# Wionerlol/MultimodalEmotionRecognition

Measured on AMD Instinct MI355X. Metric: 3s-clip train steps/sec (B=32, xattn fusion) at 1/2/4/8 MI355X, higher is better.
Workload: dtype bf16; 1 GPU; ResNet18 + WavLM-base (frozen) + xattn fusion train step (fwd+bwd+Adam); per_gpu_batch=32, global_batch=32, frames=8, image=112, audio_samples=48000, parallelism=dp1

## Files before the change

### include/mer.h

```cpp
#ifndef MER_H_
#define MER_H_

#define MER_BN_STAT_PARTS 64
#define MER_BN_STAT_ROWS(M) (((M) + 63) / 64 + 64)
#define MER_BN_RED_ROWS(M) (((M) + 63) / 64 + 4 + 64)
#define MER_BN_RED_WS_ROWS 576

#ifdef __cplusplus
extern "C" {
#endif


int mer_gemm_f32(int M, int N, int K, const void* A, int a_dtype, long sam, long sak, long bsa, const void* B,
                 int b_dtype, long sbk, long sbn, long bsb, float* C, long ldc, long bsc, const float* bias, int beta,
                 int act, int splitk, int batch, float* workspace, void* stream);

#define MER_COLSUM_WS_FLOATS(M, N) ((long)(((M) + 15) / 16) * (N))
int mer_colsum_f32(int M, int N, const float* X, long ldx, float* out, float* workspace, void* stream);

int mer_mha_fwd(int B, int H, int Lq, int Lk, int dh, const float* Q, long ldq, const float* K, long ldk,
                const float* V, long ldv, const float* bias, float* O, long ldo, float* P, float scale, float drop_p,
                const unsigned long long* seed, unsigned long long site, void* stream);

int mer_mha_bwd(int B, int H, int Lq, int Lk, int dh, const float* Q, long ldq, const float* K, long ldk,
// ... 162 lines not shown


int mer_conv_fwd(int N, int H, int W, int C, int K, int R, int S, int stride, int pad, const void* x,
                 const void* w_packed, void* y, float* stats, void* stream);

int mer_conv_fwd_ex(int N, int H, int W, int C, int K, int R, int S, int stride, int pad, const void* x,
                    const void* w_packed, void* y, float* stats, int variant, void* stream);

int mer_conv_dgrad(int N, int H, int W, int C, int K, int R, int S, int stride, int pad, const void* dy,
                   const void* wt_packed, void* dx, const void* residual, const void* residual_mask, void* stream);
int mer_conv_dgrad_ex(int N, int H, int W, int C, int K, int R, int S, int stride, int pad, const void* dy,
                      const void* wt_packed, void* dx, const void* residual, const void* residual_mask, int variant,
                      void* stream);

int mer_conv_dgrad_bnr(int N, int H, int W, int C, int K, int R, int S, int stride, int pad, const void* dy,
                       const void* wt_packed, void* dx, const void* residual, const void* residual_mask,
                       const void* bn_mask, const void* bn_x, const float* bn_ms, float* bn_red, const void* bn_x2,
                       const float* bn_ms2, float* bn_red2, int variant, void* stream);
int mer_conv_dgrad_ds(int N, int H, int W, int C, int K, int R, int S, int stride, int pad, const void* dy,
                      const void* wt_packed, void* dx, const void* residual, const void* residual_mask,
                      const void* bn_mask, const void* bn_x, const float* bn_ms, float* bn_red, const void* bn_x2,
                      const float* bn_ms2, float* bn_red2, const void* ds_dy, const void* ds_wt_packed, int ds_K,
                      int variant, void* stream);

int mer_conv_fwd_rows(int N, int H, int W, int C, int K, int R, int S, int stride, int pad, const void* x,
                      const void* w_packed, int variant);
int mer_conv_dgrad_rows(int N, int H, int W, int C, int K, int R, int S, int stride, int pad, const void* dy,
                        const void* wt_packed, const void* ds_dy, int variant);

int mer_partials_sum(int C, int parts, float* in, float* out, void* stream);
int mer_partials_sum2(int C, int parts, float* in, float* out, float* in2, float* out2, void* stream);

int mer_conv_wgrad(int N, int H, int W, int C, int Creal, int K, int R, int S, int stride, int pad, const void* x,
                   const void* dy, float* dw, int splits, float* workspace, void* stream);
int mer_conv_wgrad_ex(int N, int H, int W, int C, int Creal, int K, int R, int S, int stride, int pad, const void* x,
                      const void* dy, float* dw, int splits, float* workspace, int variant, void* stream);
int mer_conv_wgrad_partials(int N, int H, int W, int C, int K, int R, int S, int stride, int pad, const void* x,
                            const void* dy, int splits, float* workspace, int variant, void* stream);
int mer_wgrad_fold_batch(int n, const long long* rows, void* stream);

int mer_pack_input_nhwc(int N, int C, int H, int W, int Cp, const float* x, void* y, void* stream);
int mer_pack_input_s2d(int N, int C, int H, int W, const float* x, void* y, void* stream);

int mer_pack_conv_weight(int K, int C, int R, int S, int Cp, int transpose, const float* w, void* out, void* stream);

int mer_pack_conv_weights(int n, const long long* desc, long total, void* stream);
// ... 139 lines not shown
```

### multimodalemotionrecognition_amd/csrc/bn_pool.hip

```cpp
#include "common.h"
#include "mer.h"

typedef __attribute__((ext_vector_type(4))) uint32_t u32x4;

__global__ __launch_bounds__(256) void bn_stat_rows_fold_kernel(int C2, int rows, int per, const float* __restrict__ in,
                                                                float* __restrict__ out) {
  __shared__ float part[4][64];
  const int el = threadIdx.x & 63, pg = threadIdx.x >> 6;
  const int e = blockIdx.x * 64 + el, grp = blockIdx.y;
  const int r0 = grp * per, r1 = min(rows, r0 + per);
  const int ec = e < C2 ? e : C2 - 1;
  const int n = r1 - (r0 + pg) > 0 ? (r1 - (r0 + pg) + 3) / 4 : 0;
  float a0 = 0.f, a1 = 0.f;
  for (int i0 = 0; i0 < n; i0 += 16) {
    float x[16];
#pragma unroll
    for (int i = 0; i < 16; ++i) {
      const int r = r0 + pg + 4 * (i0 + i);
      x[i] = in[(long)(r < r1 ? r : r1 - 1) * C2 + ec];
    }
#pragma unroll
    for (int i = 0; i < 16; i += 2) {
      if (i0 + i < n) a0 += x[i];
      if (i0 + i + 1 < n) a1 += x[i + 1];
// ... 565 lines not shown
        float* db = h ? dbeta2 : dbeta;
        if (dg) dg[c] += rd[2 * c + 1];
        if (db) db[c] += rd[2 * c];
      }
      const float mu = m[2 * c], rs = m[2 * c + 1], gr = (h ? gamma2 : gamma)[c] * rs;
      const float a = batch_stats ? rd[2 * c] * invM : 0.f;
      const float b = batch_stats ? rd[2 * c + 1] * invM : 0.f;
      const float t = gr * b * rs;
      coef[3 * h + 0][c] = gr;
      coef[3 * h + 1][c] = -t;
      coef[3 * h + 2][c] = fmaf(-gr, a, t * mu);
    }
  }
  __syncthreads();
  const long nvec = M * C / 8;
  const long stride = (long)gridDim.x * blockDim.x;
  const long tid0 = blockIdx.x * (long)blockDim.x + threadIdx.x;
  const int c0 = (int)(tid0 % (C / 8)) * 8;
  float k[6][8];
#pragma unroll
  for (int j = 0; j < 6; ++j)
#pragma unroll
    for (int i = 0; i < 8; ++i) k[j][i] = coef[j][c0 + i];
  for (long e = tid0; e < nvec; e += stride) {
    const u32x4 gv = *reinterpret_cast<const u32x4*>(dy + e * 8);
    const u32x4 mv = *reinterpret_cast<const u32x4*>(mask + e * 8);
    const u32x4 xv = *reinterpret_cast<const u32x4*>(x + e * 8);
    const u32x4 x2v = *reinterpret_cast<const u32x4*>(x2 + e * 8);
    const bf16_t* gh = reinterpret_cast<const bf16_t*>(&gv);
    const bf16_t* mh = reinterpret_cast<const bf16_t*>(&mv);
    const bf16_t* xh = reinterpret_cast<const bf16_t*>(&xv);
    const bf16_t* x2h = reinterpret_cast<const bf16_t*>(&x2v);
    u32x4 ov, o2v;
    bf16_t* oh = reinterpret_cast<bf16_t*>(&ov);
    bf16_t* o2h = reinterpret_cast<bf16_t*>(&o2v);
#pragma unroll
    for (int i = 0; i < 8; ++i) {
      const float g = bf2f(mh[i]) > 0.f ? bf2f(gh[i]) : 0.f;
      oh[i] = f2bf(fmaf(k[0][i], g, fmaf(k[1][i], bf2f(xh[i]), k[2][i])));
      o2h[i] = f2bf(fmaf(k[3][i], g, fmaf(k[4][i], bf2f(x2h[i]), k[5][i])));
    }
    *reinterpret_cast<u32x4*>(dx + e * 8) = ov;
    *reinterpret_cast<u32x4*>(dx2 + e * 8) = o2v;
  }
}
MER_API int mer_bn_bwd_apply2(long M, int C, const void* dy, const void* mask, const void* x, const float* ms,
                              const float* gamma, const float* red, const void* x2, const float* ms2,
                              const float* gamma2, const float* red2, int batch_stats, void* dx, void* dx2,
                              float* dgamma, float* dbeta, float* dgamma2, float* dbeta2, void* stream) {
  if (C % 8 || C > 512 || 256 % (C / 8) || !mask || !x2 || !dx2 || dx == dy || dx2 == dy)
    return (int)hipErrorInvalidValue;
  const long nvec = M * C / 8;
  const int grid = bn_stream_grid(nvec);
  hipLaunchKernelGGL(bn_bwd_apply2_kernel, dim3(grid), dim3(256), 0, (hipStream_t)stream, M, C, (const bf16_t*)dy,
                     (const bf16_t*)mask, (const bf16_t*)x, ms, gamma, red, (const bf16_t*)x2, ms2, gamma2, red2,
                     batch_stats, (bf16_t*)dx, (bf16_t*)dx2, dgamma, dbeta, dgamma2, dbeta2);
  MER_LAUNCH_CHECK();
}

__global__ void maxpool_fwd_kernel(int N, int H, int W, int C, int Ho, int Wo, const bf16_t* __restrict__ x,
                                   bf16_t* __restrict__ y, uint8_t* __restrict__ arg) {
  const int cpr = C / 8;
  const int total = N * Ho * Wo * cpr;
  const float inv_cpr = 1.f / cpr, inv_Wo = 1.f / Wo, inv_Ho = 1.f / Ho;
  for (int e = blockIdx.x * blockDim.x + threadIdx.x; e < total; e += gridDim.x * blockDim.x) {
    const int q = fdiv(e, inv_cpr);
    const int c0 = (e - q * cpr) * 8;
    const int q2 = fdiv(q, inv_Wo);
    const int ow = q - q2 * Wo;
    const int n = fdiv(q2, inv_Ho);
    const int oh = q2 - n * Ho;
    float best[8];
    int bi[8];
// ... 10 lines not shown
          const float f = bf2f(vh[i]);
          if (f > best[i]) { best[i] = f; bi[i] = r * 3 + s; }
        }
      }
    u32x4 o;
    bf16_t* oh8 = reinterpret_cast<bf16_t*>(&o);
    uint2 a;
    uint8_t* a8 = reinterpret_cast<uint8_t*>(&a);
#pragma unroll
    for (int i = 0; i < 8; ++i) { oh8[i] = f2bf(best[i]); a8[i] = (uint8_t)bi[i]; }
    *reinterpret_cast<u32x4*>(y + (long)q * C + c0) = o;
    *reinterpret_cast<uint2*>(arg + (long)q * C + c0) = a;
  }
}
MER_API int mer_maxpool_fwd(int N, int H, int W, int C, const void* x, void* y, void* argmax, void* stream) {
  const int Ho = (H + 2 - 3) / 2 + 1, Wo = (W + 2 - 3) / 2 + 1;
  if (C % 8 || (long)N * H * W >= (1L << 22)) return (int)hipErrorInvalidValue;
  const long total = (long)N * Ho * Wo * C / 8;
  const int grid = (int)((total + 255) / 256 < 8192 ? (total + 255) / 256 : 8192);
  hipLaunchKernelGGL(maxpool_fwd_kernel, dim3(grid), dim3(256), 0, (hipStream_t)stream, N, H, W, C, Ho, Wo,
                     (const bf16_t*)x, (bf16_t*)y, (uint8_t*)argmax);
  MER_LAUNCH_CHECK();
}
__global__ void maxpool_bwd_kernel(int N, int H, int W, int C, int Ho, int Wo, const bf16_t* __restrict__ dy,
                                   const uint8_t* __restrict__ arg, bf16_t* __restrict__ dx) {
  const int cpr = C / 8;
  const int total = N * H * W * cpr;
  const float inv_cpr = 1.f / cpr, inv_W = 1.f / W, inv_H = 1.f / H;
  for (int e = blockIdx.x * blockDim.x + threadIdx.x; e < total; e += gridDim.x * blockDim.x) {
    const int q = fdiv(e, inv_cpr);
    const int c0 = (e - q * cpr) * 8;
    const int q2 = fdiv(q, inv_W);
    const int w = q - q2 * W;
    const int n = fdiv(q2, inv_H);
    const int h = q2 - n * H;
    float acc[8] = {0.f, 0.f, 0.f, 0.f, 0.f, 0.f, 0.f, 0.f};
    u32x4 gq[2][2];
    uint2 aq[2][2];
    int tap[2][2];
#pragma unroll
    for (int a = 0; a < 2; ++a)
#pragma unroll
      for (int b = 0; b < 2; ++b) {
        const int oh = (h + 1) / 2 - 1 + a, ow = (w + 1) / 2 - 1 + b;
        const int r = h - (oh * 2 - 1), s = w - (ow * 2 - 1);
        const bool ok = oh >= 0 && oh < Ho && ow >= 0 && ow < Wo && r >= 0 && r <= 2 && s >= 0 && s <= 2;
        const int ohc = oh < 0 ? 0 : (oh >= Ho ? Ho - 1 : oh), owc = ow < 0 ? 0 : (ow >= Wo ? Wo - 1 : ow);
        const long oi = (((long)n * Ho + ohc) * Wo + owc) * C + c0;
        gq[a][b] = *reinterpret_cast<const u32x4*>(dy + oi);
        aq[a][b] = *reinterpret_cast<const uint2*>(arg + oi);
        tap[a][b] = ok ? r * 3 + s : -1;
      }
#pragma unroll
    for (int a = 0; a < 2; ++a)
#pragma unroll
      for (int b = 0; b < 2; ++b) {
        const bf16_t* gh = reinterpret_cast<const bf16_t*>(&gq[a][b]);
        const uint8_t* a8 = reinterpret_cast<const uint8_t*>(&aq[a][b]);
#pragma unroll
        for (int i = 0; i < 8; ++i)
          if ((int)a8[i] == tap[a][b]) acc[i] += bf2f(gh[i]);
      }
    u32x4 o;
    bf16_t* oh8 = reinterpret_cast<bf16_t*>(&o);
#pragma unroll
    for (int i = 0; i < 8; ++i) oh8[i] = f2bf(acc[i]);
    *reinterpret_cast<u32x4*>(dx + (long)q * C + c0) = o;
  }
}
MER_API int mer_maxpool_bwd(int N, int H, int W, int C, const void* dy, const void* argmax, void* dx, void* stream) {
  const int Ho = (H + 2 - 3) / 2 + 1, Wo = (W + 2 - 3) / 2 + 1;
  if (C % 8 || (long)N * H * W >= (1L << 22)) return (int)hipErrorInvalidValue;
  const long total = (long)N * H * W * C / 8;
  const int grid = (int)((total + 255) / 256 < 8192 ? (total + 255) / 256 : 8192);
  hipLaunchKernelGGL(maxpool_bwd_kernel, dim3(grid), dim3(256), 0, (hipStream_t)stream, N, H, W, C, Ho, Wo,
                     (const bf16_t*)dy, (const uint8_t*)argmax, (bf16_t*)dx);
  MER_LAUNCH_CHECK();
}


__global__ void stem_bnrelu_maxpool_kernel(int N, int H, int W, int C, int Ho, int Wo, const bf16_t* __restrict__ x,
                                           const float* __restrict__ ms, const float* __restrict__ gamma,
                                           const float* __restrict__ beta, bf16_t* __restrict__ y,
                                           uint8_t* __restrict__ arg) {
  const int cpr = C / 8;
  const int total = N * Ho * Wo * cpr;
  const float inv_cpr = 1.f / cpr, inv_Wo = 1.f / Wo, inv_Ho = 1.f / Ho;
  for (int e = blockIdx.x * blockDim.x + threadIdx.x; e < total; e += gridDim.x * blockDim.x) {
    const int q = fdiv(e, inv_cpr);
// ... 30 lines not shown
    }
    u32x4 o;
    bf16_t* oh8 = reinterpret_cast<bf16_t*>(&o);
    uint2 a;
    uint8_t* a8 = reinterpret_cast<uint8_t*>(&a);
#pragma unroll
    for (int i = 0; i < 8; ++i) { oh8[i] = f2bf(best[i]); a8[i] = (uint8_t)bi[i]; }
    *reinterpret_cast<u32x4*>(y + (long)q * C + c0) = o;
    *reinterpret_cast<uint2*>(arg + (long)q * C + c0) = a;
  }
}

MER_API int mer_stem_bnrelu_maxpool_fwd(int N, int H, int W, int C, const void* x, const float* ms, const float* gamma,
                                        const float* beta, void* y, void* argmax, void* stream) {
  const int Ho = (H + 2 - 3) / 2 + 1, Wo = (W + 2 - 3) / 2 + 1;
  if (C % 8 || C > 512 || (long)N * H * W >= (1L << 22)) return (int)hipErrorInvalidValue;
  const long total = (long)N * Ho * Wo * C / 8;
  const int grid = (int)((total + 255) / 256 < 8192 ? (total + 255) / 256 : 8192);
  hipLaunchKernelGGL(stem_bnrelu_maxpool_kernel, dim3(grid), dim3(256), 0, (hipStream_t)stream, N, H, W, C, Ho, Wo,
                     (const bf16_t*)x, ms, gamma, beta, (bf16_t*)y, (uint8_t*)argmax);
  MER_LAUNCH_CHECK();
}

MER_API int mer_stem_pool_bn_bwd(int N, int H, int W, int C, const void* dy, const void* argmax, const void* x,
                                 const float* ms, const float* gamma, const float* beta, float* red, int batch_stats,
                                 void* dx, float* dgamma, float* dbeta, float* workspace, void* stream) {
  if (C % 8 || C > 512 || 256 % (C / 8) || (long)N * H * W >= (1L << 22)) return (int)hipErrorInvalidValue;
  const hipStream_t st = (hipStream_t)stream;
  const long M = (long)N * H * W;
  int rc = mer_maxpool_bwd(N, H, W, C, dy, argmax, dx, stream);
  if (rc) return rc;
  const long rpb = bn_bwd_reduce_rpb(M);
  const int blocks = (int)((M + rpb - 1) / rpb);
  hipLaunchKernelGGL((bn_bwd_reduce_kernel<true>), dim3((unsigned)blocks), dim3(256), 0, st, M, C, (const bf16_t*)dx,
                     (const bf16_t*)nullptr, (const bf16_t*)x, ms, gamma, beta, workspace, rpb);
  rc = partials_fold(C, blocks, workspace, red, st);
  if (rc) return rc;
  hipLaunchKernelGGL((bn_bwd_apply_kernel<true>), dim3(bn_stream_grid(M * C / 8)), dim3(256), 0, st, M, C,
                     (const bf16_t*)dx, (const bf16_t*)nullptr, (const bf16_t*)x, ms, gamma, beta, red, batch_stats,
                     (bf16_t*)dx, dgamma, dbeta);
  MER_LAUNCH_CHECK();
}

__global__ void avgpool_fwd_kernel(int N, int HW, int C, const bf16_t* __restrict__ x, float* __restrict__ y) {
  const int n = blockIdx.y, c = blockIdx.x * blockDim.x + threadIdx.x;
  if (c >= C) return;
  float s = 0.f;
  for (int p = 0; p < HW; ++p) s += bf2f(x[((long)n * HW + p) * C + c]);
  y[(long)n * C + c] = s / HW;
}
__global__ void avgpool_bwd_kernel(int N, int HW, int C, const float* __restrict__ dy, bf16_t* __restrict__ dx) {
  const int n = blockIdx.y;
  for (int e = blockIdx.x * blockDim.x + threadIdx.x; e < HW * C; e += gridDim.x * blockDim.x) {
    const int c = e % C;
    dx[(long)n * HW * C + e] = f2bf(dy[(long)n * C + c] / HW);
  }
}
MER_API int mer_avgpool_fwd(int N, int HW, int C, const void* x, float* y, void* stream) {
  hipLaunchKernelGGL(avgpool_fwd_kernel, dim3((C + 255) / 256, N), dim3(256), 0, (hipStream_t)stream, N, HW, C,
// ... 9 lines not shown
```

### multimodalemotionrecognition_amd/csrc/conv.hip

```cpp
#include "conv_common.h"
#include "mer.h"

MER_CT_BUFFER(mer_ct, 512 * 64)
MER_CT_BUFFER(mer_ctp, 4096 * 8)
#define CT(k) CT_AT(mer_ct_buf, k)
#define CTP(k) CTP_AT(mer_ctp_buf, k)

namespace {

template <bool DGRAD>
__device__ __forceinline__ u32x4 conv_a_chunk(const ConvGeom& g, int n, int oh, int ow, bool rowok, int kk, int tap,
                                              int c, int r, int s) {
  u32x4 v = {0u, 0u, 0u, 0u};
  if (!rowok || kk >= g.Kred) return v;
  int ih, iw;
  if (!DGRAD) {
    ih = oh * g.st - g.pad + r;
    iw = ow * g.st - g.pad + s;
  } else {
    const int th = oh + g.pad - r, tw = ow + g.pad - s;
    if (th < 0 || tw < 0) return v;
    if (g.st == 1) {
      ih = th;
      iw = tw;
// ... 395 lines not shown
        const long e0 = out_row(row) * g.ldy + colv;
        const int q = (i0 / GI) * E::PPG + rr / RPP;
        if (DGRAD && g.R_) {
          u32x4 rv, mv;
          if constexpr (PREF) {
            rv = pre->r[q];
            mv = g.Rmask ? pre->m[q] : u32x4{1u, 1u, 1u, 1u};
          } else {
            rv = *reinterpret_cast<const u32x4*>(g.R_ + e0);
            mv = g.Rmask ? *reinterpret_cast<const u32x4*>(g.Rmask + e0) : u32x4{1u, 1u, 1u, 1u};
          }
          const bf16_t* rh = reinterpret_cast<const bf16_t*>(&rv);
          const bf16_t* mh = reinterpret_cast<const bf16_t*>(&mv);
#pragma unroll
          for (int e = 0; e < 8; ++e)
            if (!g.Rmask || bf2f(mh[e]) > 0.f) v[e] += bf2f(rh[e]);
        }
        u32x4 ov;
        bf16_t* oh = reinterpret_cast<bf16_t*>(&ov);
#pragma unroll
        for (int e = 0; e < 8; ++e) {
          oh[e] = f2bf(v[e]);
          v[e] = bf2f(oh[e]);
        }
        if constexpr (DEFER) {
          pend[q] = ov;
          pend_at[q] = e0;
          pend_ok[q] = true;
        } else {
          *reinterpret_cast<u32x4*>(g.Y + e0) = ov;
        }
        if (do_bnr) {
          u32x4 mv, xv, x2v;
          if constexpr (PREF) {
            mv = pre->bm[q];
            xv = pre->x[q];
            x2v = pre->x2[q];
          } else {
            mv = *reinterpret_cast<const u32x4*>(g.bnr_mask + e0);
            xv = *reinterpret_cast<const u32x4*>(g.bnr_x + e0);
            x2v = has_x2 ? *reinterpret_cast<const u32x4*>(g.bnr_x2 + e0) : u32x4{0u, 0u, 0u, 0u};
          }
          const bf16_t* mh = reinterpret_cast<const bf16_t*>(&mv);
          const bf16_t* xh = reinterpret_cast<const bf16_t*>(&xv);
          const bf16_t* x2h = reinterpret_cast<const bf16_t*>(&x2v);
#pragma unroll
// ... 1027 lines not shown
  return mer_conv_dgrad_ex(N, H, W, C, K, R, S, stride, pad, dy, wt_packed, dx, residual, residual_mask, -1, stream);
}

MER_API int mer_conv_dgrad_ex(int N, int H, int W, int C, int K, int R, int S, int stride, int pad, const void* dy,
                              const void* wt_packed, void* dx, const void* residual, const void* residual_mask,
                              int variant, void* stream) {
  return mer_conv_dgrad_bnr(N, H, W, C, K, R, S, stride, pad, dy, wt_packed, dx, residual, residual_mask, nullptr,
                            nullptr, nullptr, nullptr, nullptr, nullptr, nullptr, variant, stream);
}

MER_API int mer_conv_dgrad_bnr(int N, int H, int W, int C, int K, int R, int S, int stride, int pad, const void* dy,
                               const void* wt_packed, void* dx, const void* residual, const void* residual_mask,
                               const void* bn_mask, const void* bn_x, const float* bn_ms, float* bn_red,
                               const void* bn_x2, const float* bn_ms2, float* bn_red2, int variant, void* stream) {
  return mer_conv_dgrad_ds(N, H, W, C, K, R, S, stride, pad, dy, wt_packed, dx, residual, residual_mask, bn_mask, bn_x,
                           bn_ms, bn_red, bn_x2, bn_ms2, bn_red2, nullptr, nullptr, 0, variant, stream);
}

MER_API int mer_conv_dgrad_ds(int N, int H, int W, int C, int K, int R, int S, int stride, int pad, const void* dy,
                              const void* wt_packed, void* dx, const void* residual, const void* residual_mask,
                              const void* bn_mask, const void* bn_x, const float* bn_ms, float* bn_red,
                              const void* bn_x2, const float* bn_ms2, float* bn_red2, const void* ds_dy,
                              const void* ds_wt_packed, int ds_K, int variant, void* stream) {
  if (K % 8 || C % 8 || variant < -1 || variant > 7) return (int)hipErrorInvalidValue;
  if (ds_dy && (stride != 2 || R != 3 || S != 3 || pad != 1 || !ds_wt_packed || ds_K <= 0 || ds_K % 64 || K % 64 ||
                variant == 0))
    return (int)hipErrorInvalidValue;
  if (bn_red && (!bn_mask || !bn_x || !bn_ms || (bn_x2 && (!bn_ms2 || !bn_red2)))) return (int)hipErrorInvalidValue;
  if (bn_red && (variant == 0 || stride > 2)) return (int)hipErrorInvalidValue;
  ConvGeom g = dgrad_geom(N, H, W, C, K, R, S, stride, pad, dy, wt_packed, ds_dy);
  g.Y = (bf16_t*)dx;
  g.R_ = (const bf16_t*)residual; g.Rmask = (const bf16_t*)residual_mask;
  g.bnr_mask = (const bf16_t*)bn_mask; g.bnr_x = (const bf16_t*)bn_x; g.bnr_ms = bn_ms; g.bnr_red = bn_red;
  g.bnr_x2 = (const bf16_t*)bn_x2; g.bnr_ms2 = bn_ms2; g.bnr_red2 = bn_red2;
  g.Wt2 = (const bf16_t*)ds_wt_packed; g.K2 = ds_dy ? ds_K : 0;
  return launch_conv_plan<true>(g, conv_plan(g, true, variant), (hipStream_t)stream);
}
```

### multimodalemotionrecognition_amd/csrc/conv_common.h

```cpp
#pragma once
#include <type_traits>

#include "common.h"
#include "mer.h"

typedef __attribute__((ext_vector_type(4))) uint32_t u32x4;
typedef __attribute__((ext_vector_type(4))) short s16x4;

#ifdef MER_CONV_TIMING
#define MER_CT_BUFFER(name, words) \
  static __device__ long long name##_buf[words]; \
  MER_API int name##_reset() { \
    static long long zeros[words]; \
    return (int)hipMemcpyToSymbol(HIP_SYMBOL(name##_buf), zeros, sizeof(zeros), 0, hipMemcpyHostToDevice); \
  } \
  MER_API int name##_read(long long* host) { \
    return (int)hipMemcpyFromSymbol(host, HIP_SYMBOL(name##_buf), sizeof(long long) * (words), 0, \
                                    hipMemcpyDeviceToHost); \
  }
#define MER_CT_MODE_WORD(name) \
  static __device__ int name##_v; \
  MER_API int name(int mode) { \
    return (int)hipMemcpyToSymbol(HIP_SYMBOL(name##_v), &mode, sizeof(int), 0, hipMemcpyHostToDevice); \
  }
// ... 21 lines not shown

constexpr int CBK = 64;

struct ConvGeom {
  int N, OH, OW;
  int IH, IW, IC;
  int R, S, st, pad;
  int Ncols;
  int Kred;
  const bf16_t* X;
  const bf16_t* Wt;
  bf16_t* Y;
  long ldy;
  float* stats;
  const bf16_t* R_;
  const bf16_t* Rmask;
  const bf16_t* bnr_mask;
  const bf16_t* bnr_x;
  const float* bnr_ms;
  float* bnr_red;
  const bf16_t* bnr_x2;
  const float* bnr_ms2;
  float* bnr_red2;
  int vec;
  const bf16_t* X2;
  const bf16_t* Wt2;
  int K2;
};

__host__ __device__ inline bool conv_vec_ok(const ConvGeom& g) {
  const uintptr_t a = (uintptr_t)g.Y | (uintptr_t)g.R_ | (uintptr_t)g.Rmask | (uintptr_t)g.bnr_mask |
                      (uintptr_t)g.bnr_x | (uintptr_t)g.bnr_x2 | (uintptr_t)g.stats | (uintptr_t)g.bnr_red |
                      (uintptr_t)g.bnr_red2;
  return g.Ncols % 8 == 0 && g.ldy % 8 == 0 && (a & 15) == 0;
}

static __device__ __attribute__((aligned(16))) uint32_t mer_conv_zero16[4] = {0u, 0u, 0u, 0u};

int cu_count() {
  static const int n = [] {
    int dev = 0, v = 0;
    if (hipGetDevice(&dev) != hipSuccess || hipDeviceGetAttribute(&v, hipDeviceAttributeMultiprocessorCount, dev) !=
                                                hipSuccess || v <= 0)
      return 256;
    return v;
  }();
// ... 5 lines not shown
```

### multimodalemotionrecognition_amd/kernels.py

```python
from __future__ import annotations

import os

import torch

from ._lib import LIB, MerKernelError

F32, BF16 = 0, 1
ACT = {"none": 0, "relu": 1, "gelu": 2}


def stream_ptr() -> int:
    return torch.cuda.current_stream().cuda_stream


class KernelProbe:

    def __init__(self, name: str, key: tuple, units: float):
        self.name, self.key, self.units = name, tuple(key), units
        self.pairs = []
        self.active = False

    def matches(self, name, key):
        return self.active and name == self.name and tuple(key) == self.key
# ... 424 lines not shown
    if stats is not None:
        return _partial_rows("mer_conv_fwd_rows", N, H, W, C, Kc, R, S, stride, pad, x.data_ptr(), wp.data_ptr(),
                             int(variant))
    return None


_ROWS_CACHE = {}
PARTIAL_ROWS = True


def _partial_rows(fn, *args):
    if not PARTIAL_ROWS:
        return None
    key = (fn,) + tuple(a % 16 == 0 if isinstance(a, int) and a > 1 << 20 else a for a in args)
    r = _ROWS_CACHE.get(key)
    if r is None:
        r = int(LIB.call_int(fn, *args))
        if r <= 0:
            raise MerKernelError(f"{fn}{args[:9]} failed: {r}")
        _ROWS_CACHE[key] = r
    return r


def conv_dgrad(dy, wt, dx, R, S, stride, pad, residual=None, mask=None, variant=-1, bnr=None, ds=None):
    N, H, W, C = dx.shape
    Kc = dy.shape[-1]
    Ho, Wo = (H + 2 * pad - R) // stride + 1, (W + 2 * pad - S) // stride + 1
    if tuple(dy.shape) != (N, Ho, Wo, Kc) or tuple(wt.shape) != (C, R * S * Kc):
        raise ValueError(f"conv_dgrad shapes dy{tuple(dy.shape)} wt{tuple(wt.shape)} dx{tuple(dx.shape)}")
    b = list(bnr) + [None] * (7 - len(bnr)) if bnr is not None else [None] * 7
    for t in (b[0], b[1], b[4]):
        if t is not None and tuple(t.shape) != tuple(dx.shape):
            raise ValueError("conv_dgrad bnr tensors must match dx")
    for t in (b[3], b[6]):
        if t is not None and t.numel() != bn_red_rows(N * H * W) * C * 2:
            raise ValueError("conv_dgrad bnr red buffers must be zeroed [bn_red_rows(N*H*W), C, 2]")
    if ds is not None:
        ddy, dwt = ds
        Kd = ddy.shape[-1]
        if tuple(ddy.shape) != (N, Ho, Wo, Kd) or tuple(dwt.shape) != (C, Kd) or stride != 2 or R != 3 or pad != 1:
            raise ValueError("conv_dgrad ds: a 1x1 / stride-2 downsample gradient beside a 3x3 / stride-2 / pad-1 conv")
        _launch("conv_dgrad", (N, H, W, C, Kc, R, stride), "mer_conv_dgrad_ds", N, H, W, C, Kc, R, S, stride, pad,
                dy.data_ptr(), wt.data_ptr(), dx.data_ptr(), _ptr(residual), _ptr(mask), *[_ptr(t) for t in b],
                ddy.data_ptr(), dwt.data_ptr(), Kd, int(variant), stream_ptr())
    else:
        _launch("conv_dgrad", (N, H, W, C, Kc, R, stride), "mer_conv_dgrad_bnr", N, H, W, C, Kc, R, S, stride, pad,
                dy.data_ptr(), wt.data_ptr(), dx.data_ptr(), _ptr(residual), _ptr(mask), *[_ptr(t) for t in b],
                int(variant), stream_ptr())
    if bnr is None:
        return None
    return _partial_rows("mer_conv_dgrad_rows", N, H, W, C, Kc, R, S, stride, pad, dy.data_ptr(), wt.data_ptr(),
                         ds[0].data_ptr() if ds is not None else 0, int(variant))


def partials_sum(parts_buf, out, rows=None):
    P, C, _ = parts_buf.shape
    if P <= 64:
        raise ValueError("partials_sum expects a bn_red_rows(M) buffer (data rows + 64 scratch rows)")
    if rows is None:
        rows = P - 64
    if not 0 < rows <= P - 64:
        raise ValueError("partials_sum rows out of range")
    LIB("mer_partials_sum", C, int(rows), parts_buf.data_ptr(), out.data_ptr(), stream_ptr())
    return out
# ... 145 lines not shown
    LIB("mer_bn_apply", M, C, x.data_ptr(), ms.data_ptr(), gamma.data_ptr(), beta.data_ptr(), _ptr(res), _ptr(ms2),
        _ptr(gamma2), _ptr(beta2), int(relu), y.data_ptr(), stream_ptr())


def bn_bwd_reduce(dy, mask, x, ms, red, workspace=None):
    C = x.shape[-1]
    if workspace is None:
        workspace = torch.empty(BN_RED_WS_ROWS * C * 2, device=x.device, dtype=torch.float32)
    if workspace.numel() < BN_RED_WS_ROWS * C * 2:
        raise ValueError("bn_bwd_reduce workspace too small")
    LIB("mer_bn_bwd_reduce", x.numel() // C, C, dy.data_ptr(), _ptr(mask), x.data_ptr(), ms.data_ptr(),
        red.data_ptr(), workspace.data_ptr(), stream_ptr())


def bn_bwd_apply(dy, mask, x, ms, gamma, red, dx, dgamma, dbeta, batch_stats=True):
    C = x.shape[-1]
    LIB("mer_bn_bwd_apply", x.numel() // C, C, dy.data_ptr(), _ptr(mask), x.data_ptr(), ms.data_ptr(),
        gamma.data_ptr(), red.data_ptr(), int(batch_stats), dx.data_ptr(), _ptr(dgamma), _ptr(dbeta), stream_ptr())


def bn_bwd_apply2(dy, mask, x, ms, gamma, red, dx, dgamma, dbeta, x2, ms2, gamma2, red2, dx2, dgamma2, dbeta2,
                  batch_stats=True):
    C = x.shape[-1]
    for t in (dy, mask, x2, dx, dx2):
        if tuple(t.shape) != tuple(x.shape):
            raise ValueError("bn_bwd_apply2 tensors must share one shape")
    LIB("mer_bn_bwd_apply2", x.numel() // C, C, dy.data_ptr(), mask.data_ptr(), x.data_ptr(), ms.data_ptr(),
        gamma.data_ptr(), red.data_ptr(), x2.data_ptr(), ms2.data_ptr(), gamma2.data_ptr(), red2.data_ptr(),
        int(batch_stats), dx.data_ptr(), dx2.data_ptr(), _ptr(dgamma), _ptr(dbeta), _ptr(dgamma2), _ptr(dbeta2),
        stream_ptr())


def maxpool_fwd(x, y, arg):
    N, H, W, C = x.shape
    LIB("mer_maxpool_fwd", N, H, W, C, x.data_ptr(), y.data_ptr(), arg.data_ptr(), stream_ptr())


def stem_bnrelu_maxpool(x, ms, gamma, beta, y, arg):
    N, H, W, C = x.shape
    LIB("mer_stem_bnrelu_maxpool_fwd", N, H, W, C, x.data_ptr(), ms.data_ptr(), gamma.data_ptr(), beta.data_ptr(),
        y.data_ptr(), arg.data_ptr(), stream_ptr())


def stem_pool_bn_bwd(dy, arg, x, ms, gamma, beta, red, dx, dgamma, dbeta, batch_stats=True, workspace=None):
    N, H, W, C = x.shape
    if workspace is None:
        workspace = torch.empty(BN_RED_WS_ROWS * C * 2, device=x.device, dtype=torch.float32)
    if workspace.numel() < BN_RED_WS_ROWS * C * 2:
        raise ValueError("stem_pool_bn_bwd workspace too small")
    LIB("mer_stem_pool_bn_bwd", N, H, W, C, dy.data_ptr(), arg.data_ptr(), x.data_ptr(), ms.data_ptr(),
# ... 444 lines not shown
```

### multimodalemotionrecognition_amd/video.py

```python
from __future__ import annotations

import os
import warnings
from typing import List

import torch
from torch import nn

from . import graphs as G
from . import kernels as K
from .nn_ops import hip_linear
from .optim import weight_version
from .temporal import TemporalPooler

S2D_CH = 16


class BasicBlock(nn.Module):
    expansion = 1

    def __init__(self, inplanes: int, planes: int, stride: int = 1, downsample: nn.Module = None):
        super().__init__()
        self.conv1 = nn.Conv2d(inplanes, planes, 3, stride, 1, bias=False)
        self.bn1 = nn.BatchNorm2d(planes)
# ... 445 lines not shown
def _block_bwd_floats(sv) -> int:
    xin, bc1, _, ba1, bc2, _, _, _, out = sv
    C1, C2, Cin = bc1.shape[-1], bc2.shape[-1], xin.shape[-1]
    return 2 * (K.bn_red_rows(ba1.numel() // C1) * C1 + 2 * K.BN_RED_WS_ROWS * C2 + C2 * 2
                + 2 * K.bn_red_rows(xin.numel() // Cin) * Cin)


def _bnr_target(blk_sv, blk, arena):
    xin, bc1, bms1, ba1, bc2, bms2, cd, msd, out = blk_sv
    C2 = bc2.shape[-1]
    rows = K.bn_red_rows(out.numel() // C2)
    red2 = arena.take(C2, parts=rows)
    if cd is None:
        return (out, bc2, bms2, red2), (red2, None)
    redd = arena.take(C2, parts=rows)
    return (out, bc2, bms2, red2, cd, msd, redd), (red2, redd)


WGRAD_DEFER = True
BN_BWD_PAIR = True
BN_FIN_PAIR = True
FOLD_EVERY = 2
FUSED_DS_DGRAD = True


class _WgradLane:

    def __init__(self, device):
        self.folds = K.WgradFolds() if WGRAD_DEFER else None

    def run(self, fn, *reads, block=None):
        fn()

    def join(self):
        if self.folds is not None:
            self.folds.flush()


@torch.no_grad()
def block_backward(trunk, blk: BasicBlock, sv, dx: torch.Tensor, grads, training: bool = True, pre=None,
                   prev=None, arena=None, lane=None, bidx=None):
    dev = dx.device
    xin, bc1, bms1, ba1, bc2, bms2, cd, msd, out = sv
    if arena is None:
        arena = _StatsArena(trunk, dev, floats=_block_bwd_floats(sv))
    own_lane = lane is None
    if own_lane:
        lane = _WgradLane(dev)
    g_out = dx
    s = blk.stride
    C2 = bc2.shape[-1]
    if pre is not None:
        if cd is not None and BN_FIN_PAIR:
            red2, redd = K.partials_sum_pair(pre[0], torch.empty(C2, 2, device=dev, dtype=torch.float32), pre[1],
                                             torch.empty(C2, 2, device=dev, dtype=torch.float32), pre[2])
        else:
            red2 = K.partials_sum(pre[0], torch.empty(C2, 2, device=dev, dtype=torch.float32), pre[2])
            redd = K.partials_sum(pre[1], torch.empty(C2, 2, device=dev, dtype=torch.float32), pre[2]) \
                if cd is not None else None
    else:
        red2 = arena.take(C2, parts=1)
        K.bn_bwd_reduce(g_out, out, bc2, bms2, red2, arena.take(C2, parts=K.BN_RED_WS_ROWS))
        redd = None
        if cd is not None:
            redd = arena.take(C2, parts=1)
            K.bn_bwd_reduce(g_out, out, cd, msd, redd, arena.take(C2, parts=K.BN_RED_WS_ROWS))
    if cd is not None and BN_BWD_PAIR:
        dc2, dcd = torch.empty_like(bc2), torch.empty_like(cd)
        bd = blk.downsample[1]
        K.bn_bwd_apply2(g_out, out, bc2, bms2, blk.bn2.weight, red2, dc2, _grad(blk.bn2.weight, grads),
                        _grad(blk.bn2.bias, grads), cd, msd, bd.weight, redd, dcd, _grad(bd.weight, grads),
                        _grad(bd.bias, grads), training)
    else:
        dc2 = _bn_bwd(g_out, out, bc2, bms2, blk.bn2, red2, grads, training)
        dcd = _bn_bwd(g_out, out, cd, msd, blk.downsample[1], redd, grads, training) if cd is not None else None
    w2 = _grad(blk.conv2.weight, grads)
    if w2 is not None:
        lane.run(lambda: K.conv_wgrad(ba1, dc2, w2, 3, 3, 1, 1, defer=lane.folds), ba1, dc2, w2, block=bidx)
    da1 = torch.empty_like(ba1)
    C1 = bc1.shape[-1]
    red1p = arena.take(C1, parts=K.bn_red_rows(ba1.numel() // C1))
    rows1 = K.conv_dgrad(dc2, trunk.packed(blk.conv2, C2, True), da1, 3, 3, 1, 1, bnr=(ba1, bc1, bms1, red1p))
    red1 = K.partials_sum(red1p, torch.empty(C1, 2, device=dev, dtype=torch.float32), rows1)
    dc1 = _bn_bwd(da1, ba1, bc1, bms1, blk.bn1, red1, grads, training)
    w1 = _grad(blk.conv1.weight, grads)
    if w1 is not None:
        lane.run(lambda: K.conv_wgrad(xin, dc1, w1, 3, 3, s, 1, defer=lane.folds), xin, dc1, w1, block=bidx)
    dxin = torch.empty_like(xin)
    Cin = xin.shape[-1]
    bnr, nxt = _bnr_target(prev[0], prev[1], arena) if prev is not None else (None, None)
    if cd is not None:
        wd = _grad(blk.downsample[0].weight, grads)
        if wd is not None:
            lane.run(lambda: K.conv_wgrad(xin, dcd, wd, 1, 1, s, 0, defer=lane.folds), xin, dcd, wd, block=bidx)
        if FUSED_DS_DGRAD and s == 2:
            rows = K.conv_dgrad(dc1, trunk.packed(blk.conv1, Cin, True), dxin, 3, 3, s, 1, bnr=bnr,
                                ds=(dcd, trunk.packed(blk.downsample[0], Cin, True)))
        else:
            dxd = torch.empty_like(xin)
            K.conv_dgrad(dcd, trunk.packed(blk.downsample[0], Cin, True), dxd, 1, 1, s, 0)
            rows = K.conv_dgrad(dc1, trunk.packed(blk.conv1, Cin, True), dxin, 3, 3, s, 1, residual=dxd, bnr=bnr)
    else:
        rows = K.conv_dgrad(dc1, trunk.packed(blk.conv1, Cin, True), dxin, 3, 3, s, 1, residual=g_out, mask=out,
                            bnr=bnr)
    if own_lane:
        lane.join()
    return dxin, (nxt + (rows,) if nxt is not None else None)


@torch.no_grad()
def trunk_backward(trunk: ResNet18Trunk, saved, dfeat: torch.Tensor, training: bool = True, force_pack: bool = False,
                   hook=None):
    split = SPLIT_BLOCK if hook is not None else 0
    state = trunk_backward_start(trunk, saved, dfeat, training, split, force_pack=force_pack)
    if hook is not None:
        hook(trunk.split_params(split))
    return trunk_backward_finish(trunk, saved, state, training, force_pack=force_pack)


@torch.no_grad()
def trunk_backward_start(trunk, saved, dfeat, training, split, force_pack=False):
    with _ForcePack(trunk, force_pack):
        trunk.pack_all(transpose=True)
        dev = dfeat.device
        x = saved["final"]
        dx = torch.empty_like(x)
        K.avgpool_bwd(dfeat, dx)
# ... 76 lines not shown
```

Before: 225.6 steps/s.

## Store ReLU-masked gradients from dgrad epilogue and fuse maxpool bwd into stem BN reduce

The conv dgrad epilogue, when fused with the BN reduction, can now zero out gradient elements where the ReLU mask is inactive before storing them. Downstream BN backward apply kernels and residual paths can then skip reading the mask tensor, since a null mask means all ones. Separately, the stem maxpool backward gather is fused into the BN reduce kernel, which removes a full pass that reread dx. The cost is extra mask reads inside the dgrad epilogue and more complex kernel plumbing, with a risk of incorrect gradients if a consumer still expects unmasked values.

```diff
diff --git a/include/mer.h b/include/mer.h
--- a/include/mer.h
+++ b/include/mer.h
@@ -208,6 +208,11 @@
                       const void* bn_mask, const void* bn_x, const float* bn_ms, float* bn_red, const void* bn_x2,
                       const float* bn_ms2, float* bn_red2, const void* ds_dy, const void* ds_wt_packed, int ds_K,
                       int variant, void* stream);
+int mer_conv_dgrad_dsm(int N, int H, int W, int C, int K, int R, int S, int stride, int pad, const void* dy,
+                       const void* wt_packed, void* dx, const void* residual, const void* residual_mask,
+                       const void* bn_mask, const void* bn_x, const float* bn_ms, float* bn_red, const void* bn_x2,
+                       const float* bn_ms2, float* bn_red2, const void* ds_dy, const void* ds_wt_packed, int ds_K,
+                       int variant, int store_masked, void* stream);
 
 int mer_conv_fwd_rows(int N, int H, int W, int C, int K, int R, int S, int stride, int pad, const void* x,
                       const void* w_packed, int variant);
diff --git a/multimodalemotionrecognition_amd/csrc/bn_pool.hip b/multimodalemotionrecognition_amd/csrc/bn_pool.hip
--- a/multimodalemotionrecognition_amd/csrc/bn_pool.hip
+++ b/multimodalemotionrecognition_amd/csrc/bn_pool.hip
@@ -611,9 +611,10 @@
   for (int j = 0; j < 6; ++j)
 #pragma unroll
     for (int i = 0; i < 8; ++i) k[j][i] = coef[j][c0 + i];
+  const u32x4 one16 = {0x3f803f80u, 0x3f803f80u, 0x3f803f80u, 0x3f803f80u};
   for (long e = tid0; e < nvec; e += stride) {
     const u32x4 gv = *reinterpret_cast<const u32x4*>(dy + e * 8);
-    const u32x4 mv = *reinterpret_cast<const u32x4*>(mask + e * 8);
+    const u32x4 mv = mask ? *reinterpret_cast<const u32x4*>(mask + e * 8) : one16;
     const u32x4 xv = *reinterpret_cast<const u32x4*>(x + e * 8);
     const u32x4 x2v = *reinterpret_cast<const u32x4*>(x2 + e * 8);
     const bf16_t* gh = reinterpret_cast<const bf16_t*>(&gv);
@@ -637,7 +638,7 @@
                               const float* gamma, const float* red, const void* x2, const float* ms2,
                               const float* gamma2, const float* red2, int batch_stats, void* dx, void* dx2,
                               float* dgamma, float* dbeta, float* dgamma2, float* dbeta2, void* stream) {
-  if (C % 8 || C > 512 || 256 % (C / 8) || !mask || !x2 || !dx2 || dx == dy || dx2 == dy)
+  if (C % 8 || C > 512 || 256 % (C / 8) || !x2 || !dx2 || dx == dy || dx2 == dy)
     return (int)hipErrorInvalidValue;
   const long nvec = M * C / 8;
   const int grid = bn_stream_grid(nvec);
@@ -694,6 +695,42 @@
                      (const bf16_t*)x, (bf16_t*)y, (uint8_t*)argmax);
   MER_LAUNCH_CHECK();
 }
+__device__ __forceinline__ u32x4 maxpool_gather8(int n, int h, int w, int C, int Ho, int Wo, int c0,
+                                                 const bf16_t* __restrict__ dy, const uint8_t* __restrict__ arg) {
+  float acc[8] = {0.f, 0.f, 0.f, 0.f, 0.f, 0.f, 0.f, 0.f};
+  u32x4 gq[2][2];
+  uint2 aq[2][2];
+  int tap[2][2];
+#pragma unroll
+  for (int a = 0; a < 2; ++a)
+#pragma unroll
+    for (int b = 0; b < 2; ++b) {
+      const int oh = (h + 1) / 2 - 1 + a, ow = (w + 1) / 2 - 1 + b;
+      const int r = h - (oh * 2 - 1), s = w - (ow * 2 - 1);
+      const bool ok = oh >= 0 && oh < Ho && ow >= 0 && ow < Wo && r >= 0 && r <= 2 && s >= 0 && s <= 2;
+      const int ohc = oh < 0 ? 0 : (oh >= Ho ? Ho - 1 : oh), owc = ow < 0 ? 0 : (ow >= Wo ? Wo - 1 : ow);
+      const long oi = (((long)n * Ho + ohc) * Wo + owc) * C + c0;
+      gq[a][b] = *reinterpret_cast<const u32x4*>(dy + oi);
+      aq[a][b] = *reinterpret_cast<const uint2*>(arg + oi);
+      tap[a][b] = ok ? r * 3 + s : -1;
+    }
+#pragma unroll
+  for (int a = 0; a < 2; ++a)
+#pragma unroll
+    for (int b = 0; b < 2; ++b) {
+      const bf16_t* gh = reinterpret_cast<const bf16_t*>(&gq[a][b]);
+      const uint8_t* a8 = reinterpret_cast<const uint8_t*>(&aq[a][b]);
+#pragma unroll
+      for (int i = 0; i < 8; ++i)
+        if ((int)a8[i] == tap[a][b]) acc[i] += bf2f(gh[i]);
+    }
+  u32x4 o;
+  bf16_t* oh8 = reinterpret_cast<bf16_t*>(&o);
+#pragma unroll
+  for (int i = 0; i < 8; ++i) oh8[i] = f2bf(acc[i]);
+  return o;
+}
+
 __global__ void maxpool_bwd_kernel(int N, int H, int W, int C, int Ho, int Wo, const bf16_t* __restrict__ dy,
                                    const uint8_t* __restrict__ arg, bf16_t* __restrict__ dx) {
   const int cpr = C / 8;
@@ -706,37 +743,7 @@
     const int w = q - q2 * W;
     const int n = fdiv(q2, inv_H);
     const int h = q2 - n * H;
-    float acc[8] = {0.f, 0.f, 0.f, 0.f, 0.f, 0.f, 0.f, 0.f};
-    u32x4 gq[2][2];
-    uint2 aq[2][2];
-    int tap[2][2];
-#pragma unroll
-    for (int a = 0; a < 2; ++a)
-#pragma unroll
-      for (int b = 0; b < 2; ++b) {
-        const int oh = (h + 1) / 2 - 1 + a, ow = (w + 1) / 2 - 1 + b;
-        const int r = h - (oh * 2 - 1), s = w - (ow * 2 - 1);
-        const bool ok = oh >= 0 && oh < Ho && ow >= 0 && ow < Wo && r >= 0 && r <= 2 && s >= 0 && s <= 2;
-        const int ohc = oh < 0 ? 0 : (oh >= Ho ? Ho - 1 : oh), owc = ow < 0 ? 0 : (ow >= Wo ? Wo - 1 : ow);
-        const long oi = (((long)n * Ho + ohc) * Wo + owc) * C + c0;
-        gq[a][b] = *reinterpret_cast<const u32x4*>(dy + oi);
-        aq[a][b] = *reinterpret_cast<const uint2*>(arg + oi);
-        tap[a][b] = ok ? r * 3 + s : -1;
-      }
-#pragma unroll
-    for (int a = 0; a < 2; ++a)
-#pragma unroll
-      for (int b = 0; b < 2; ++b) {
-        const bf16_t* gh = reinterpret_cast<const bf16_t*>(&gq[a][b]);
-        const uint8_t* a8 = reinterpret_cast<const uint8_t*>(&aq[a][b]);
-#pragma unroll
-        for (int i = 0; i < 8; ++i)
-          if ((int)a8[i] == tap[a][b]) acc[i] += bf2f(gh[i]);
-      }
-    u32x4 o;
-    bf16_t* oh8 = reinterpret_cast<bf16_t*>(&o);
-#pragma unroll
-    for (int i = 0; i < 8; ++i) oh8[i] = f2bf(acc[i]);
+    const u32x4 o = maxpool_gather8(n, h, w, C, Ho, Wo, c0, dy, arg);
     *reinterpret_cast<u32x4*>(dx + (long)q * C + c0) = o;
   }
 }
@@ -813,19 +820,94 @@
   MER_LAUNCH_CHECK();
 }
 
+__global__ __launch_bounds__(256) void stem_pool_bn_reduce_kernel(int N, int H, int W, int C, int Ho, int Wo,
+                                                                  const bf16_t* __restrict__ dy,
+                                                                  const uint8_t* __restrict__ arg,
+                                                                  const bf16_t* __restrict__ x,
+                                                                  const float* __restrict__ ms,
+                                                                  const float* __restrict__ mgamma,
+                                                                  const float* __restrict__ mbeta,
+                                                                  bf16_t* __restrict__ dx, float* __restrict__ rows,
+                                                                  long rows_per_block) {
+  __shared__ float part[2][2048];
+  const long M = (long)N * H * W;
+  const int cpr = C / 8;
+  const int rows_per_iter = 256 / cpr > 0 ? 256 / cpr : 1;
+  const int tc = threadIdx.x % cpr, tr = threadIdx.x / cpr;
+  const long r0 = blockIdx.x * rows_per_block, r1 = min(M, r0 + rows_per_block);
+  const float inv_W = 1.f / W, inv_H = 1.f / H;
+  float s1[8] = {0.f}, s2[8] = {0.f};
+  if (tr < rows_per_iter) {
+    float mean[8], rstd[8], msc[8], msh[8];
+#pragma unroll
+    for (int i = 0; i < 8; ++i) {
+      mean[i] = ms[2 * (tc * 8 + i)];
+      rstd[i] = ms[2 * (tc * 8 + i) + 1];
+      stem_bn_coef(tc * 8 + i, ms, mgamma, mbeta, msc[i], msh[i]);
+    }
+    for (long rb = r0 + tr; rb < r1; rb += 4 * rows_per_iter) {
+      u32x4 gv[4], xv[4];
+#pragma unroll
+      for (int u = 0; u < 4; ++u) {
+        const long r = rb + u * rows_per_iter;
+        const int q = (int)(r < r1 ? r : r1 - 1);
+        const int q2 = fdiv(q, inv_W);
+        const int w = q - q2 * W;
+        const int n = fdiv(q2, inv_H);
+        const int h = q2 - n * H;
+        xv[u] = *reinterpret_cast<const u32x4*>(x + (long)q * C + tc * 8);
+        gv[u] = maxpool_gather8(n, h, w, C, Ho, Wo, tc * 8, dy, arg);
+      }
+#pragma unroll
+      for (int u = 0; u < 4; ++u) {
+        const long r = rb + u * rows_per_iter;
+        const bool rowok = r < r1;
+        if (rowok) *reinterpret_cast<u32x4*>(dx + r * C + tc * 8) = gv[u];
+        const bf16_t* gh = reinterpret_cast<const bf16_t*>(&gv[u]);
+        const bf16_t* xh = reinterpret_cast<const bf16_t*>(&xv[u]);
+#pragma unroll
+        for (int i = 0; i < 8; ++i) {
+          const bool live = bf2f(f2bf(fmaxf(bf2f(xh[i]) * msc[i] + msh[i], 0.f))) > 0.f;
+          const float g = (live && rowok) ? bf2f(gh[i]) : 0.f;
+          if (rowok) {
+            s1[i] += g;
+            s2[i] += g * (bf2f(xh[i]) - mean[i]) * rstd[i];
+          }
+        }
+      }
+    }
+#pragma unroll
+    for (int i = 0; i < 8; ++i) {
+      part[0][tr * C + tc * 8 + i] = s1[i];
+      part[1][tr * C + tc * 8 + i] = s2[i];
+    }
+  }
+  __syncthreads();
+  float* out = rows + (long)blockIdx.x * C * 2;
+  for (int c = threadIdx.x; c < C; c += 256) {
+    float a = 0.f, b = 0.f;
+    for (int q = 0; q < rows_per_iter; ++q) {
+      a += part[0][q * C + c];
+      b += part[1][q * C + c];
+    }
+    out[2 * c] = a;
+    out[2 * c + 1] = b;
+  }
+}
+
 MER_API int mer_stem_pool_bn_bwd(int N, int H, int W, int C, const void* dy, const void* argmax, const void* x,
                                  const float* ms, const float* gamma, const float* beta, float* red, int batch_stats,
                                  void* dx, float* dgamma, float* dbeta, float* workspace, void* stream) {
   if (C % 8 || C > 512 || 256 % (C / 8) || (long)N * H * W >= (1L << 22)) return (int)hipErrorInvalidValue;
   const hipStream_t st = (hipStream_t)stream;
   const long M = (long)N * H * W;
-  int rc = mer_maxpool_bwd(N, H, W, C, dy, argmax, dx, stream);
-  if (rc) return rc;
+  const int Ho = (H + 2 - 3) / 2 + 1, Wo = (W + 2 - 3) / 2 + 1;
   const long rpb = bn_bwd_reduce_rpb(M);
   const int blocks = (int)((M + rpb - 1) / rpb);
-  hipLaunchKernelGGL((bn_bwd_reduce_kernel<true>), dim3((unsigned)blocks), dim3(256), 0, st, M, C, (const bf16_t*)dx,
-                     (const bf16_t*)nullptr, (const bf16_t*)x, ms, gamma, beta, workspace, rpb);
-  rc = partials_fold(C, blocks, workspace, red, st);
+  hipLaunchKernelGGL(stem_pool_bn_reduce_kernel, dim3((unsigned)blocks), dim3(256), 0, st, N, H, W, C, Ho, Wo,
+                     (const bf16_t*)dy, (const uint8_t*)argmax, (const bf16_t*)x, ms, gamma, beta, (bf16_t*)dx,
+                     workspace, rpb);
+  int rc = partials_fold(C, blocks, workspace, red, st);
   if (rc) return rc;
   hipLaunchKernelGGL((bn_bwd_apply_kernel<true>), dim3(bn_stream_grid(M * C / 8)), dim3(256), 0, st, M, C,
                      (const bf16_t*)dx, (const bf16_t*)nullptr, (const bf16_t*)x, ms, gamma, beta, red, batch_stats,
diff --git a/multimodalemotionrecognition_amd/csrc/conv.hip b/multimodalemotionrecognition_amd/csrc/conv.hip
--- a/multimodalemotionrecognition_amd/csrc/conv.hip
+++ b/multimodalemotionrecognition_amd/csrc/conv.hip
@@ -441,6 +441,17 @@
         for (int e = 0; e < 8; ++e) {
           oh[e] = f2bf(v[e]);
           v[e] = bf2f(oh[e]);
+        }
+        if (do_bnr && g.store_masked) {
+          u32x4 sv;
+          if constexpr (PREF)
+            sv = pre->bm[q];
+          else
+            sv = *reinterpret_cast<const u32x4*>(g.bnr_mask + e0);
+          const bf16_t* sh = reinterpret_cast<const bf16_t*>(&sv);
+#pragma unroll
+          for (int e = 0; e < 8; ++e)
+            if (!(bf2f(sh[e]) > 0.f)) oh[e] = 0;
         }
         if constexpr (DEFER) {
           pend[q] = ov;
@@ -1514,6 +1525,15 @@
                               const void* bn_mask, const void* bn_x, const float* bn_ms, float* bn_red,
                               const void* bn_x2, const float* bn_ms2, float* bn_red2, const void* ds_dy,
                               const void* ds_wt_packed, int ds_K, int variant, void* stream) {
+  return mer_conv_dgrad_dsm(N, H, W, C, K, R, S, stride, pad, dy, wt_packed, dx, residual, residual_mask, bn_mask, bn_x,
+                            bn_ms, bn_red, bn_x2, bn_ms2, bn_red2, ds_dy, ds_wt_packed, ds_K, variant, 0, stream);
+}
+
+MER_API int mer_conv_dgrad_dsm(int N, int H, int W, int C, int K, int R, int S, int stride, int pad, const void* dy,
+                               const void* wt_packed, void* dx, const void* residual, const void* residual_mask,
+                               const void* bn_mask, const void* bn_x, const float* bn_ms, float* bn_red,
+                               const void* bn_x2, const float* bn_ms2, float* bn_red2, const void* ds_dy,
+                               const void* ds_wt_packed, int ds_K, int variant, int store_masked, void* stream) {
   if (K % 8 || C % 8 || variant < -1 || variant > 7) return (int)hipErrorInvalidValue;
   if (ds_dy && (stride != 2 || R != 3 || S != 3 || pad != 1 || !ds_wt_packed || ds_K <= 0 || ds_K % 64 || K % 64 ||
                 variant == 0))
@@ -1526,5 +1546,7 @@
   g.bnr_mask = (const bf16_t*)bn_mask; g.bnr_x = (const bf16_t*)bn_x; g.bnr_ms = bn_ms; g.bnr_red = bn_red;
   g.bnr_x2 = (const bf16_t*)bn_x2; g.bnr_ms2 = bn_ms2; g.bnr_red2 = bn_red2;
   g.Wt2 = (const bf16_t*)ds_wt_packed; g.K2 = ds_dy ? ds_K : 0;
+  if (store_masked && (!bn_red || !g.vec || !conv_vec_ok(g))) return (int)hipErrorInvalidValue;
+  g.store_masked = store_masked != 0;
   return launch_conv_plan<true>(g, conv_plan(g, true, variant), (hipStream_t)stream);
 }
diff --git a/multimodalemotionrecognition_amd/csrc/conv_common.h b/multimodalemotionrecognition_amd/csrc/conv_common.h
--- a/multimodalemotionrecognition_amd/csrc/conv_common.h
+++ b/multimodalemotionrecognition_amd/csrc/conv_common.h
@@ -67,6 +67,7 @@
   const bf16_t* bnr_x2;
   const float* bnr_ms2;
   float* bnr_red2;
+  int store_masked;
   int vec;
   const bf16_t* X2;
   const bf16_t* Wt2;
diff --git a/multimodalemotionrecognition_amd/kernels.py b/multimodalemotionrecognition_amd/kernels.py
--- a/multimodalemotionrecognition_amd/kernels.py
+++ b/multimodalemotionrecognition_amd/kernels.py
@@ -470,7 +470,8 @@
     return r
 
 
-def conv_dgrad(dy, wt, dx, R, S, stride, pad, residual=None, mask=None, variant=-1, bnr=None, ds=None):
+def conv_dgrad(dy, wt, dx, R, S, stride, pad, residual=None, mask=None, variant=-1, bnr=None, ds=None,
+               store_masked=False):
     N, H, W, C = dx.shape
     Kc = dy.shape[-1]
     Ho, Wo = (H + 2 * pad - R) // stride + 1, (W + 2 * pad - S) // stride + 1
@@ -488,6 +489,12 @@
         Kd = ddy.shape[-1]
         if tuple(ddy.shape) != (N, Ho, Wo, Kd) or tuple(dwt.shape) != (C, Kd) or stride != 2 or R != 3 or pad != 1:
             raise ValueError("conv_dgrad ds: a 1x1 / stride-2 downsample gradient beside a 3x3 / stride-2 / pad-1 conv")
+    if store_masked:
+        _launch("conv_dgrad", (N, H, W, C, Kc, R, stride), "mer_conv_dgrad_dsm", N, H, W, C, Kc, R, S, stride, pad,
+                dy.data_ptr(), wt.data_ptr(), dx.data_ptr(), _ptr(residual), _ptr(mask), *[_ptr(t) for t in b],
+                _ptr(ds[0] if ds is not None else None), _ptr(ds[1] if ds is not None else None),
+                Kd if ds is not None else 0, int(variant), 1, stream_ptr())
+    elif ds is not None:
         _launch("conv_dgrad", (N, H, W, C, Kc, R, stride), "mer_conv_dgrad_ds", N, H, W, C, Kc, R, S, stride, pad,
                 dy.data_ptr(), wt.data_ptr(), dx.data_ptr(), _ptr(residual), _ptr(mask), *[_ptr(t) for t in b],
                 ddy.data_ptr(), dwt.data_ptr(), Kd, int(variant), stream_ptr())
@@ -679,10 +686,10 @@
 def bn_bwd_apply2(dy, mask, x, ms, gamma, red, dx, dgamma, dbeta, x2, ms2, gamma2, red2, dx2, dgamma2, dbeta2,
                   batch_stats=True):
     C = x.shape[-1]
-    for t in (dy, mask, x2, dx, dx2):
+    for t in (dy, x if mask is None else mask, x2, dx, dx2):
         if tuple(t.shape) != tuple(x.shape):
             raise ValueError("bn_bwd_apply2 tensors must share one shape")
-    LIB("mer_bn_bwd_apply2", x.numel() // C, C, dy.data_ptr(), mask.data_ptr(), x.data_ptr(), ms.data_ptr(),
+    LIB("mer_bn_bwd_apply2", x.numel() // C, C, dy.data_ptr(), _ptr(mask), x.data_ptr(), ms.data_ptr(),
         gamma.data_ptr(), red.data_ptr(), x2.data_ptr(), ms2.data_ptr(), gamma2.data_ptr(), red2.data_ptr(),
         int(batch_stats), dx.data_ptr(), dx2.data_ptr(), _ptr(dgamma), _ptr(dbeta), _ptr(dgamma2), _ptr(dbeta2),
         stream_ptr())
diff --git a/multimodalemotionrecognition_amd/video.py b/multimodalemotionrecognition_amd/video.py
--- a/multimodalemotionrecognition_amd/video.py
+++ b/multimodalemotionrecognition_amd/video.py
@@ -491,6 +491,7 @@
 BN_FIN_PAIR = True
 FOLD_EVERY = 2
 FUSED_DS_DGRAD = True
+MASKED_GRAD = True
 
 
 class _WgradLane:
@@ -517,6 +518,7 @@
     if own_lane:
         lane = _WgradLane(dev)
     g_out = dx
+    m_out = None if (MASKED_GRAD and pre is not None) else out
     s = blk.stride
     C2 = bc2.shape[-1]
     if pre is not None:
@@ -537,41 +539,44 @@
     if cd is not None and BN_BWD_PAIR:
         dc2, dcd = torch.empty_like(bc2), torch.empty_like(cd)
         bd = blk.downsample[1]
-        K.bn_bwd_apply2(g_out, out, bc2, bms2, blk.bn2.weight, red2, dc2, _grad(blk.bn2.weight, grads),
+        K.bn_bwd_apply2(g_out, m_out, bc2, bms2, blk.bn2.weight, red2, dc2, _grad(blk.bn2.weight, grads),
                         _grad(blk.bn2.bias, grads), cd, msd, bd.weight, redd, dcd, _grad(bd.weight, grads),
                         _grad(bd.bias, grads), training)
     else:
-        dc2 = _bn_bwd(g_out, out, bc2, bms2, blk.bn2, red2, grads, training)
-        dcd = _bn_bwd(g_out, out, cd, msd, blk.downsample[1], redd, grads, training) if cd is not None else None
+        dc2 = _bn_bwd(g_out, m_out, bc2, bms2, blk.bn2, red2, grads, training)
+        dcd = _bn_bwd(g_out, m_out, cd, msd, blk.downsample[1], redd, grads, training) if cd is not None else None
     w2 = _grad(blk.conv2.weight, grads)
     if w2 is not None:
         lane.run(lambda: K.conv_wgrad(ba1, dc2, w2, 3, 3, 1, 1, defer=lane.folds), ba1, dc2, w2, block=bidx)
     da1 = torch.empty_like(ba1)
     C1 = bc1.shape[-1]
     red1p = arena.take(C1, parts=K.bn_red_rows(ba1.numel() // C1))
-    rows1 = K.conv_dgrad(dc2, trunk.packed(blk.conv2, C2, True), da1, 3, 3, 1, 1, bnr=(ba1, bc1, bms1, red1p))
+    rows1 = K.conv_dgrad(dc2, trunk.packed(blk.conv2, C2, True), da1, 3, 3, 1, 1, bnr=(ba1, bc1, bms1, red1p),
+                         store_masked=MASKED_GRAD)
     red1 = K.partials_sum(red1p, torch.empty(C1, 2, device=dev, dtype=torch.float32), rows1)
-    dc1 = _bn_bwd(da1, ba1, bc1, bms1, blk.bn1, red1, grads, training)
+    dc1 = _bn_bwd(da1, None if MASKED_GRAD else ba1, bc1, bms1, blk.bn1, red1, grads, training)
     w1 = _grad(blk.conv1.weight, grads)
     if w1 is not None:
         lane.run(lambda: K.conv_wgrad(xin, dc1, w1, 3, 3, s, 1, defer=lane.folds), xin, dc1, w1, block=bidx)
     dxin = torch.empty_like(xin)
     Cin = xin.shape[-1]
     bnr, nxt = _bnr_target(prev[0], prev[1], arena) if prev is not None else (None, None)
+    sm = MASKED_GRAD and bnr is not None
     if cd is not None:
         wd = _grad(blk.downsample[0].weight, grads)
         if wd is not None:
             lane.run(lambda: K.conv_wgrad(xin, dcd, wd, 1, 1, s, 0, defer=lane.folds), xin, dcd, wd, block=bidx)
         if FUSED_DS_DGRAD and s == 2:
             rows = K.conv_dgrad(dc1, trunk.packed(blk.conv1, Cin, True), dxin, 3, 3, s, 1, bnr=bnr,
-                                ds=(dcd, trunk.packed(blk.downsample[0], Cin, True)))
+                                ds=(dcd, trunk.packed(blk.downsample[0], Cin, True)), store_masked=sm)
         else:
             dxd = torch.empty_like(xin)
             K.conv_dgrad(dcd, trunk.packed(blk.downsample[0], Cin, True), dxd, 1, 1, s, 0)
-            rows = K.conv_dgrad(dc1, trunk.packed(blk.conv1, Cin, True), dxin, 3, 3, s, 1, residual=dxd, bnr=bnr)
+            rows = K.conv_dgrad(dc1, trunk.packed(blk.conv1, Cin, True), dxin, 3, 3, s, 1, residual=dxd, bnr=bnr,
+                                store_masked=sm)
     else:
-        rows = K.conv_dgrad(dc1, trunk.packed(blk.conv1, Cin, True), dxin, 3, 3, s, 1, residual=g_out, mask=out,
-                            bnr=bnr)
+        rows = K.conv_dgrad(dc1, trunk.packed(blk.conv1, Cin, True), dxin, 3, 3, s, 1, residual=g_out, mask=m_out,
+                            bnr=bnr, store_masked=sm)
     if own_lane:
         lane.join()
     return dxin, (nxt + (rows,) if nxt is not None else None)
```

New measurement: 226.7 steps/s (median of 6 runs). Within noise of the previous version (+0.5%).
